# haoheliu/ssr_eval

Hardware: AMD Instinct MI355X
Metric: utterance-pairs/sec (LSD+SSIM, 48kHz, n_fft=2048) (higher is better)
Workload: dtype f64

## Files before the change

ssr_eval_amd/csrc/ssr_stft_wave.h:

```cpp
#pragma once
#include "ssr_stft.h"


constexpr int SSR_W_N = 2048, SSR_W_L = 64, SSR_W_P = 32;
constexpr int SSR_W_TWP = 7 * 32 + 12 * 64;
SSR_DEV int ssr_wpad(int i) { return i + (i >> 5); }
constexpr int SSR_W_PN = SSR_W_N + (SSR_W_N >> 5) + 1;

template <typename T> SSR_DEV cx<T> ssr_w32(int m) {
  constexpr double c[22] = {1.0, 0.98078528040323044913, 0.92387953251128675613, 0.83146961230254523708, 0.70710678118654752440,
                            0.55557023301960222474, 0.38268343236508977173, 0.19509032201612826785, 0.0,
                            -0.19509032201612826785, -0.38268343236508977173, -0.55557023301960222474, -0.70710678118654752440,
                            -0.83146961230254523708, -0.92387953251128675613, -0.98078528040323044913, -1.0,
                            -0.98078528040323044913, -0.92387953251128675613, -0.83146961230254523708, -0.70710678118654752440,
                            -0.55557023301960222474};
  constexpr double s[22] = {0.0, -0.19509032201612826785, -0.38268343236508977173, -0.55557023301960222474, -0.70710678118654752440,
                            -0.83146961230254523708, -0.92387953251128675613, -0.98078528040323044913, -1.0,
                            -0.98078528040323044913, -0.92387953251128675613, -0.83146961230254523708, -0.70710678118654752440,
                            -0.55557023301960222474, -0.38268343236508977173, -0.19509032201612826785, 0.0,
                            0.19509032201612826785, 0.38268343236508977173, 0.55557023301960222474, 0.70710678118654752440,
                            0.83146961230254523708};
  return {(T)c[m], (T)s[m]};
}

template <typename T, int NZ = 32> SSR_DEV void ssr_dft32(cx<T>* v) {
  const T h = (T)0.70710678118654752440;
  static_assert(NZ == 32 || (NZ > 8 && NZ <= 16), "full, or two non-zero row groups");
  SSR_UNROLL for (int n2 = 0; n2 < 8; ++n2) {
    cx<T> t[4] = {v[n2], v[8 + n2], v[16 + n2], v[24 + n2]};
    if (NZ == 32) {
      ssr_bfly4(t);
    } else if (8 + n2 < NZ) {
      const cx<T> r = cmul_negi(t[1]);
      t[2] = csub(t[0], t[1]); t[3] = csub(t[0], r);
      t[1] = cadd(t[0], r);    t[0] = cadd(t[0], v[8 + n2]);
    } else {
      t[1] = t[0]; t[2] = t[0]; t[3] = t[0];
    }
    SSR_UNROLL for (int k1 = 0; k1 < 4; ++k1) {
      const int m = n2 * k1;
      cx<T> x = t[k1];
      if (m == 0) {
      } else if (m == 8) {
        x = cmul_negi(x);
      } else if (m == 16) {
        x = {-x.x, -x.y};
      } else if (m == 4) {
        x = {h * (x.x + x.y), h * (x.y - x.x)};
      } else if (m == 12) {
        x = {h * (x.y - x.x), -h * (x.x + x.y)};
      } else if (m == 20) {
        x = {-h * (x.x + x.y), h * (x.x - x.y)};
      } else {
        x = cmul(x, ssr_w32<T>(m));
      }
      v[8 * k1 + n2] = x;
    }
  }
  SSR_UNROLL for (int k1 = 0; k1 < 4; ++k1) ssr_bfly8(v + 8 * k1);
}
SSR_DEV constexpr int ssr_dft32_freq(int rho) { return (rho >> 3) + 4 * (rho & 7); }

struct SsrTrue { static constexpr bool value = true; };
struct SsrFalse { static constexpr bool value = false; };

template <typename T, bool SUMS> struct SsrWaveRegs {
  cx<T> v[SSR_W_P];
  T tx[SSR_W_P];
  float pa[SSR_W_P], pb[SSR_W_P];
  T wl[SSR_W_P / 2];
  cx<T> tw1[7];
  cx<T> tw2[12];
  double lsd_total;
};

template <typename T, bool SPLIT> struct SsrWaveLds {
  static constexpr size_t bytes() { return sizeof(double) * 4 + sizeof(int) * 8 + sizeof(T) * (SPLIT ? 1 : 2) * SSR_W_PN; }
  double* sc1; int* nz; T* re; T* im;
  SSR_MEMBER explicit SsrWaveLds(char* base) {
    sc1 = reinterpret_cast<double*>(base);
    nz = reinterpret_cast<int*>(sc1 + 4);
    re = reinterpret_cast<T*>(nz + 8);
    im = SPLIT ? re : re + SSR_W_PN;
  }
  SSR_MEMBER bool nonzero(int which, int par) const {
    int f = nz[which * 2 + par];
#ifndef SSR_HOST_EMU
    f = __builtin_amdgcn_readfirstlane(f);
#endif
    return f != 0;
  }
};

template <typename T> struct SsrWaveBuf { T* re; T* im; };

template <typename T, bool SPLIT> constexpr size_t ssr_stft_wave_sums_offset() { return (SsrWaveLds<T, SPLIT>::bytes() + 7) & ~(size_t)7; }
template <typename T, bool SPLIT, bool SUMS> constexpr size_t ssr_stft_wave_lds_bytes() {
  return SUMS ? ssr_stft_wave_sums_offset<T, SPLIT>() + 6 * 64 * sizeof(double) : SsrWaveLds<T, SPLIT>::bytes();
}

struct SsrWaveBase { int st0, ld8, st1; };
SSR_DEV SsrWaveBase ssr_wave_bases(int tid) {
  return {33 * tid, tid + (tid >> 5), 264 * (tid >> 5) + (tid & 31)};
}
SSR_DEV constexpr int ssr_w_off_st0(int i) { return ssr_dft32_freq(i); }
SSR_DEV constexpr int ssr_w_off_ld8(int i) { return 66 * (i >> 3) + 264 * (i & 7); }
SSR_DEV constexpr int ssr_w_off_st1(int i) { return 528 * (i >> 3) + 33 * (i & 7); }

#define SSR_W_EXCHANGE_G(blk, regs, L, WB, WO, RBASES, RIDX, EXTRA)                                       \
  if constexpr (!SPLIT) {                                                                                 \
    SSR_WPHASE(blk, regs, { const int w_ = ssr_wave_bases(tid & 63).WB;                                        \
      SSR_UNROLL for (int i = 0; i < SSR_W_P; ++i) { (L).re[w_ + WO(i)] = R.v[i].x; (L).im[w_ + WO(i)] = R.v[i].y; } }); \
    SSR_WPHASE(blk, regs, { SSR_SCHED_BARRIER(); EXTRA; const auto r_ = RBASES(tid & 63);                    \
      SSR_UNROLL for (int i = 0; i < SSR_W_P; ++i) R.v[i] = {(L).re[RIDX(r_, i)], (L).im[RIDX(r_, i)]}; });   \
  } else {                                                                                                \
    SSR_WPHASE(blk, regs, { const int w_ = ssr_wave_bases(tid & 63).WB;                                        \
      SSR_UNROLL for (int i = 0; i < SSR_W_P; ++i) (L).re[w_ + WO(i)] = R.v[i].x; });                     \
    SSR_WPHASE(blk, regs, { SSR_SCHED_BARRIER(); EXTRA; const auto r_ = RBASES(tid & 63);                    \
      SSR_UNROLL for (int i = 0; i < SSR_W_P; ++i) R.tx[i] = (L).re[RIDX(r_, i)]; });                     \
    SSR_WPHASE(blk, regs, { const int w_ = ssr_wave_bases(tid & 63).WB;                                        \
      SSR_UNROLL for (int i = 0; i < SSR_W_P; ++i) (L).re[w_ + WO(i)] = R.v[i].y; });                     \
    SSR_WPHASE(blk, regs, { const auto r_ = RBASES(tid & 63);                                                \
      SSR_UNROLL for (int i = 0; i < SSR_W_P; ++i) R.v[i] = {R.tx[i], (L).re[RIDX(r_, i)]}; });           \
  }
#define SSR_W_RIDX_LD8(b_, i) ((b_).ld8 + ssr_w_off_ld8(i))
#define SSR_W_EXCHANGE(blk, regs, L, WB, WO, RB, RO, EXTRA) SSR_W_EXCHANGE_G(blk, regs, L, WB, WO, ssr_wave_bases, SSR_W_RIDX_##RB##_##RO, EXTRA)
#define SSR_W_RIDX_ld8_ssr_w_off_ld8(b_, i) SSR_W_RIDX_LD8(b_, i)

struct SsrWavePBase { int ld8, p2, p3; };
SSR_DEV int ssr_wave_pj3(int tid) { return tid == 0 ? 128 : 256 - tid; }
SSR_DEV SsrWavePBase ssr_wave_pbases(int tid) {
  return {tid + (tid >> 5), ssr_wpad(192 - tid), ssr_wpad(ssr_wave_pj3(tid))};
}
SSR_DEV int ssr_w_rd_paired(const SsrWavePBase& B, int i) {
  const int b = i >> 3, q = i & 7;
  return (b == 0 ? B.ld8 : b == 1 ? B.ld8 + 66 : b == 2 ? B.p2 : B.p3) + 264 * q;
}
#define SSR_W_RIDX_PAIRED(b_, i) ssr_w_rd_paired(b_, i)
#define SSR_W_LOAD_TW2_PAIRED { const int t_ = tid & 63; const unsigned l_ = SSR_UIDX(t_);                       \
    const unsigned o2_ = SSR_UIDX(t_ == 0 ? 192 : 64 - t_); const unsigned o3_ = SSR_UIDX(t_ == 0 ? -192 : 64 - t_); \
    SSR_UNROLL for (int i = 0; i < 6; ++i) R.tw2[i] = VT.at(l_ + (SSR_W_N + 224 + 64 * i));                       \
    SSR_UNROLL for (int i = 6; i < 9; ++i) R.tw2[i] = VT.at(o2_ + (SSR_W_N + 224 + 64 * i));                      \
    SSR_UNROLL for (int i = 9; i < 12; ++i) R.tw2[i] = VT.at(o3_ + (SSR_W_N + 224 + 64 * i)); }

#define SSR_W_LOAD_TW1 { const unsigned l_ = SSR_UIDX(tid & 31); \
                         SSR_UNROLL for (int q = 1; q < 8; ++q) R.tw1[q - 1] = VT.at(l_ + (SSR_W_N + 32 * (q - 1))); }
#define SSR_W_LOAD_TW2 { const unsigned l_ = SSR_UIDX(tid & 63); \
                         SSR_UNROLL for (int i = 0; i < 12; ++i) R.tw2[i] = VT.at(l_ + (SSR_W_N + 224 + 64 * i)); }
#define SSR_W_FFT_TAIL(blk, BLK0, regs, L, EXTRA2)                                                                        \
  SSR_W_FFT_TAIL_X(blk, BLK0, regs, L, SSR_W_EXCHANGE(blk, regs, L, st1, ssr_w_off_st1, ld8, ssr_w_off_ld8, SSR_W_LOAD_TW2 EXTRA2))
#define SSR_W_FFT_TAIL_PAIRED(blk, BLK0, regs, L)                                                                         \
  SSR_W_FFT_TAIL_X(blk, BLK0, regs, L, SSR_W_EXCHANGE_G(blk, regs, L, st1, ssr_w_off_st1, ssr_wave_pbases, SSR_W_RIDX_PAIRED, SSR_W_LOAD_TW2_PAIRED))
#define SSR_W_FFT_TAIL_X(blk, BLK0, regs, L, EXCH2)                                                                       \
  blk = BLK0; ssr_launder(blk);                                                                                     \
  SSR_W_EXCHANGE(blk, regs, L, st0, ssr_w_off_st0, ld8, ssr_w_off_ld8, SSR_W_LOAD_TW1);                             \
   \
  SSR_WPHASE(blk, regs, {                                                                                           \
    SSR_UNROLL for (int b = 0; b < 4; ++b) {                                                                        \
      SSR_UNROLL for (int q = 1; q < 8; ++q) R.v[8 * b + q] = cmul(R.v[8 * b + q], R.tw1[q - 1]);                   \
      ssr_bfly8(R.v + 8 * b);                                                                                       \
    }                                                                                                               \
  });                                                                                                               \
  blk = BLK0; ssr_launder(blk);                                                                                     \
  EXCH2;                                                                                                            \
    \
  SSR_WPHASE(blk, regs, {                                                                                           \
    SSR_UNROLL for (int b = 0; b < 4; ++b) {                                                                        \
      cx<T>* x = R.v + 8 * b;                                                                                       \
      const cx<T> w1 = R.tw2[3 * b], w2 = R.tw2[3 * b + 1], w4 = R.tw2[3 * b + 2];                                  \
      x[1] = cmul(x[1], w1);                                                                                        \
      x[2] = cmul(x[2], w2);                                                                                        \
      x[4] = cmul(x[4], w4);                                                                                        \
      const cx<T> w3 = cmul(w1, w2);                                                                                \
      x[3] = cmul(x[3], w3);                                                                                        \
      x[5] = cmul(x[5], cmul(w1, w4));                                                                              \
      x[6] = cmul(x[6], cmul(w2, w4));                                                                              \
      x[7] = cmul(x[7], cmul(w3, w4));                                                                              \
      ssr_bfly8(x);                                                                                                 \
    }                                                                                                               \
  });

template <typename T, int WHICH = 3, typename REGS>
SSR_DEV void ssr_wave_prefetch(const SsrStftParams<T>& p, REGS& R, int tid, const SsrView<float>& va, const SsrView<float>& vb,
                               int u, int n, int n_frames) {
  const int t_c = (u < n_frames) ? u : n_frames - 1;
  const int base = t_c * p.hop - SSR_W_N / 2;
  if (base >= 0 && base + SSR_W_N <= n) {
    SSR_UNROLL for (int r = 0; r < SSR_W_P; ++r) {
      if (WHICH & 1) R.pa[r] = va.at(SSR_UIDX(tid + 64 * r), base);
      if (WHICH & 2) R.pb[r] = vb.at(SSR_UIDX(tid + 64 * r), base);
    }
  } else {
    SSR_UNROLL for (int r = 0; r < SSR_W_P; ++r) {
      const unsigned m = SSR_UIDX(ssr_reflect(base + tid + 64 * r, n));
      if (WHICH & 1) R.pa[r] = va.at(m);
      if (WHICH & 2) R.pb[r] = vb.at(m);
    }
  }
}

template <typename REGS> SSR_DEV void ssr_wave_flags(REGS& R, int tid, int* nz, int par) {
  SSR_UNROLL for (int r = 0; r < SSR_W_P; ++r) { ssr_touch(R.pa[r]); ssr_touch(R.pb[r]); }
  unsigned ora = 0u, orb = 0u;
  SSR_UNROLL for (int r = 1; r < SSR_W_P; ++r) { ora |= ssr_mag_bits(R.pa[r]); orb |= ssr_mag_bits(R.pb[r]); }
  ora |= (tid == 0) ? 0u : ssr_mag_bits(R.pa[0]);
  orb |= (tid == 0) ? 0u : ssr_mag_bits(R.pb[0]);
  SSR_WAVE_ANY_STORE(tid, ora != 0u, nz + par);
  SSR_WAVE_ANY_STORE(tid, orb != 0u, nz + 2 + par);
}

template <typename T, bool SUMS, bool SPLIT, int MAG = -1, typename BLK>
SSR_BODY void ssr_stft_wave_body(const SsrStftParams<T>& p, BLK& blk, int chunk, int item, char* lds_base) {
  constexpr int N = SSR_W_N, F = N / 2 + 1;
  using Regs = SsrWaveRegs<T, SUMS>;
  SsrWaveLds<T, SPLIT> L(lds_base);
  const int n = p.len[item], hop = p.hop;
  const int n_frames = ssr_num_frames_dev(n, N, hop);
  const int S = p.interleave > 1 ? p.interleave : 1;
  const int span0 = (chunk / S) * S * p.units_per_chunk;
  const int u0 = span0 + chunk % S;
  const int u1 = (span0 + S * p.units_per_chunk < n_frames) ? span0 + S * p.units_per_chunk : n_frames;
  const float* sa = p.a + p.a_off[item];
  const float* sb = p.b + p.b_off[item];
  const int64_t row0 = p.frame_off[item];
  double* part = p.part ? p.part + ((int64_t)item * p.n_chunks + chunk) * SSR_NPART : nullptr;
  const int mask = SUMS ? p.metric_mask : (p.metric_mask & SSR_M_LSD);
  const bool want_lsd = mask & SSR_M_LSD;
  const SsrView<float> va(sa, n), vb(sb, n);
  const SsrView<T> vw(p.window, N);
  const SsrView<cx<T>> vt(p.tw, N + SSR_W_TWP);

  double* lsum = reinterpret_cast<double*>(lds_base + ssr_stft_wave_sums_offset<T, SPLIT>());
  SSR_REGS(Regs, regs, blk);
  SSR_WPHASE(blk, regs, {
    R.lsd_total = 0.0;
    if constexpr (SUMS) for (int q = 0; q < 6; ++q) lsum[64 * q + tid] = 0.0;
    if (tid == 0) L.sc1[0] = 0.0;
    if (u0 < u1) {
      ssr_wave_prefetch<T>(p, R, tid, va, vb, u0, n, n_frames);
      SSR_UNROLL for (int r = 0; r < SSR_W_P / 2; ++r) R.wl[r] = vw.at(SSR_UIDX(tid + 64 * r));
    }
    SSR_VMEM_DRAIN();
  });

  BLK blk0 = blk;
  for (int u = u0, it = 0; u < u1; u += S, ++it) {
    blk = blk0; ssr_launder(blk);
    SSR_WPHASE(blk, regs, {
      ssr_wave_flags(R, tid, L.nz, it & 1);
      SSR_UNROLL for (int r = 0; r < SSR_W_P; ++r) {
        const T w = (r < SSR_W_P / 2) ? R.wl[r] : (T)0.5 - R.wl[r - SSR_W_P / 2];
        R.v[r] = {(T)R.pa[r] * w, (T)R.pb[r] * w};
      }
      ssr_dft32(R.v);
      if (want_lsd && it > 0 && tid == 0) R.lsd_total += sqrt(L.sc1[0] / (double)F);
    });
#define VT vt
    SSR_W_FFT_TAIL_PAIRED(blk, blk0, regs, L);
#undef VT

    blk = blk0; ssr_launder(blk);
    const int64_t OP = p.out_pitch ? p.out_pitch : F;
    float* ra0 = p.out_a ? p.out_a + (row0 + u) * OP : nullptr;
    float* rb0 = p.out_b ? p.out_b + (row0 + u) * OP : nullptr;
    SSR_WPHASE(blk, regs, {
      SSR_SCHED_BARRIER();
      double acc[7] = {0.0, 0.0, 0.0, 0.0, 0.0, 0.0, 0.0};
      const int par = it & 1;
      const bool a_nz = L.nonzero(0, par), b_nz = L.nonzero(1, par);
      const bool both = a_nz && b_nz;
      const bool store = MAG < 0 ? p.out_kind == SSR_OUT_MAG : MAG != 0;
      const SsrRwView<float> wa(ra0, store ? F : 0), wb(rb0, (store && rb0 != nullptr) ? F : 0);
      const int lane4 = 4 * tid, lane4_2 = 4 * (192 - tid), lane4_3 = 4 * ssr_wave_pj3(tid);
      auto bin_off = [&](int b, int q) -> int {
        return (b == 0 ? lane4 : b == 1 ? lane4 + 256 : b == 2 ? lane4_2 : lane4_3) + 1024 * q;
      };
      cx<T> rot4 = {(T)0, (T)0};
      if (tid == 0) {
        rot4 = R.v[28];
        const cx<T> t29 = R.v[29], t30 = R.v[30], t31 = R.v[31];
        R.v[31] = R.v[0]; R.v[30] = R.v[7]; R.v[29] = R.v[6]; R.v[28] = R.v[5];
        R.v[7] = t31; R.v[6] = t30; R.v[5] = t29;
      }
      constexpr int G = 2;
      constexpr int PF1 = SUMS ? 1 : 0;
      auto bins = [&](auto fast_tag) {
        constexpr bool FAST = decltype(fast_tag)::value;
        SSR_UNROLL for (int b = 0; b < 4; ++b) SSR_UNROLL for (int q0 = 0; q0 < 4; q0 += G) {
          cx<T> zn[G];
          SSR_UNROLL for (int q = 0; q < G; ++q) zn[q] = R.v[8 * (3 - b) + 7 - (q0 + q)];
          SSR_UNROLL for (int q = 0; q < G; q += 2) {
            const cx<T> zk0 = R.v[8 * b + q0 + q], zk1 = R.v[8 * b + q0 + q + 1];
            f2 e, t;
            if constexpr (FAST) {
              ssr_pair_bins2_fast<T, SUMS>(acc, zk0, zn[q], zk1, zn[q + 1], e, t);
            } else {
              float e0, t0, e1, t1;
              ssr_pair_bin<T, 0, true>(mask, acc, zk0, zn[q], a_nz, b_nz, e0, t0);
              ssr_pair_bin<T, 0, true>(mask, acc, zk1, zn[q + 1], a_nz, b_nz, e1, t1);
              e = f2_make(e0, e1); t = f2_make(t0, t1);
            }
            if (store) {
              wa.st_raw(bin_off(b, q0 + q), e.x);
              wa.st_raw(bin_off(b, q0 + q + 1), e.y);
              wb.st_raw(bin_off(b, q0 + q), t.x);
              wb.st_raw(bin_off(b, q0 + q + 1), t.y);
            }
          }
          if (b == 0 && q0 + G == 4) {
            if (tid == 0) {
              const cx<T> zq = R.v[4];
              float e, t;
              ssr_pair_bin<T, 0, true>(mask, acc, zq, zq, a_nz, b_nz, e, t);
              if (store) { wa.st_raw(4 * (N / 2), e); wb.st_raw(4 * (N / 2), t); }
              R.v[4] = rot4;
            }
          }
          if (b == PF1 && q0 + G == 4) {
            SSR_SCHED_BARRIER();
            ssr_wave_prefetch<T, 1>(p, R, tid, va, vb, u + S, n, n_frames);
            SSR_SCHED_BARRIER();
          }
          if (b == PF1 + 1 && q0 + G == 4) {
            SSR_SCHED_BARRIER();
            ssr_wave_prefetch<T, 2>(p, R, tid, va, vb, u + S, n, n_frames);
            SSR_SCHED_BARRIER();
          }
          if (b == PF1 + 2 && q0 + G == 4) {
            SSR_SCHED_BARRIER();
            SSR_UNROLL for (int r = 0; r < SSR_W_P / 2; ++r) R.wl[r] = vw.at(SSR_UIDX(tid + 64 * r));
            SSR_SCHED_BARRIER();
          }
        }
      };
      constexpr int FULL = SUMS ? (SSR_M_LSD | SSR_M_LOG_SISPEC | SSR_M_SISPEC) : SSR_M_LSD;
      if (both && (mask & 7) == FULL) bins(SsrTrue{});
      else bins(SsrFalse{});
      if (want_lsd) SSR_WAVE_SUM_STORE(tid, 64, acc[0], L.sc1);
      if constexpr (SUMS)
        for (int q = 0; q < 6; ++q) SSR_LDS_ACCUM(lsum + 64 * q + tid, acc[1 + q]);
    });
  }

  if (part == nullptr) return;
  if constexpr (SUMS) {
    for (int q = 0; q < 6; ++q) {
      SSR_WPHASE(blk, regs, SSR_WAVE_SUM_STORE(tid, 64, lsum[64 * q + tid], L.sc1 + 1));
      SSR_WPHASE(blk, regs, if (tid == 0) part[1 + q] = L.sc1[1]);
    }
  } else {
    SSR_WPHASE(blk, regs, if (tid == 0) for (int q = 0; q < 6; ++q) part[1 + q] = 0.0);
  }
  SSR_WPHASE(blk, regs, if (tid == 0) {
    double lsd = R.lsd_total;
    if (want_lsd && u1 > u0) lsd += sqrt(L.sc1[0] / (double)F);
    part[0] = lsd;
    part[7] = 0.0;
  });
}
```

ssr_eval_amd/csrc/tu_stft.inc:

```
#include "ssr_host.h"
#include "ssr_stft_r3.h"
#include "ssr_stft_wave.h"
#include "ssr_stft_rn_wave.h"
#include "ssr_stft_r3_rot.h"

typedef SSR_TU_T TT;
static_assert(SSR_W_N == SSR_WAVE_N && SSR_W_TWP == SSR_WAVE_TWP, "ssr_tables.h appends what ssr_stft_wave.h reads");
static_assert(SSR_W24_N == SSR_WAVE24_N && SSR_W24_TWP == SSR_WAVE24_TWP, "ssr_tables.h appends what ssr_fft24.h reads");

constexpr int ssr_stft_min_waves(int logn, bool blu, bool sums) { return (logn == 11 && !blu && !sums) ? 4 : 1; }

#if SSR_TU_PART <= 2
template <typename T, int LOGN, bool BLU, int MODE, bool SUMS, int E64>
__global__ __launch_bounds__((1 << LOGN) / ssr_stft_ppt(LOGN, BLU), E64 ? 1 : ssr_stft_min_waves(LOGN, BLU, SUMS))
void k_stft(SsrStftParams<T> p) {
  extern __shared__ __attribute__((aligned(16))) char smem[];
  SsrBlk blk{(int)threadIdx.x};
  const int item = blockIdx.x / p.n_chunks, chunk = blockIdx.x % p.n_chunks;
  ssr_stft_body<T, LOGN, BLU, MODE, SUMS, ssr_stft_ppt(LOGN, BLU), E64>(p, blk, chunk, item, smem);
}

template <typename T, int LOGN, bool BLU, int MODE, bool SUMS, int E64 = 0>
static int launch_stft_mode(SsrStftParams<T>& p, int grid, hipStream_t s) {
  constexpr int PPT = ssr_stft_ppt(LOGN, BLU);
  const size_t lds = SsrStftLds<T, LOGN, PPT>::bytes();
  static thread_local SsrLdsSlot slot;
  if (int rc = ssr_allow_lds((const void*)k_stft<T, LOGN, BLU, MODE, SUMS, E64>, lds, &slot)) return rc;
  hipLaunchKernelGGL((k_stft<T, LOGN, BLU, MODE, SUMS, E64>), dim3(grid), dim3((1 << LOGN) / PPT), lds, s, p);
  HIP_TRY(hipGetLastError());
  return SSR_OK;
}

template <typename T, int LOGN, bool BLU> static int launch_stft_inst(SsrStftParams<T>& p, int grid, hipStream_t s) {
  const bool sums = p.metric_mask & (SSR_M_SISPEC | SSR_M_LOG_SISPEC);
  (void)sums;
#if SSR_TU_PART == 2
  return launch_stft_mode<T, LOGN, BLU, SSR_MODE_SINGLE, false>(p, grid, s);
#elif SSR_TU_PART == 1
  if (p.a64 && p.b64)
    return sums ? launch_stft_mode<T, LOGN, BLU, SSR_MODE_PAIR, true, SSR_IN_BOTH64>(p, grid, s)
                : launch_stft_mode<T, LOGN, BLU, SSR_MODE_PAIR, false, SSR_IN_BOTH64>(p, grid, s);
  return sums ? launch_stft_mode<T, LOGN, BLU, SSR_MODE_PAIR, true, SSR_IN_EST64>(p, grid, s)
              : launch_stft_mode<T, LOGN, BLU, SSR_MODE_PAIR, false, SSR_IN_EST64>(p, grid, s);
#else
  return sums ? launch_stft_mode<T, LOGN, BLU, SSR_MODE_PAIR, true>(p, grid, s)
              : launch_stft_mode<T, LOGN, BLU, SSR_MODE_PAIR, false>(p, grid, s);
#endif
}

#if SSR_TU_PART == 0
template <typename T, bool SUMS, bool SPLIT, bool MAG>
__global__ __launch_bounds__(64, SPLIT ? 2 : 1) void k_stft_wave(SsrStftParams<T> p, int n_groups) {
  extern __shared__ __attribute__((aligned(16))) char smem[];
  SsrBlk blk{(int)threadIdx.x};
  int logical = (int)blockIdx.x;
  if (p.interleave > 1) {
    const int S = p.interleave, xcd = (int)blockIdx.x & 7, slot = (int)blockIdx.x >> 3;
    const int G = (slot / S) * 8 + xcd;
    if (G >= n_groups) return;
    logical = G * S + slot % S;
  }
  const int item = logical / p.n_chunks, chunk = logical % p.n_chunks;
  ssr_stft_wave_body<T, SUMS, SPLIT, MAG ? 1 : 0>(p, blk, chunk, item, smem);
}
template <typename T, bool SUMS> static int launch_stft_wave(SsrStftParams<T>& p, int grid, hipStream_t s) {
  const size_t lds = ssr_stft_wave_lds_bytes<T, true, SUMS>();
  int n_groups = grid;
  if (p.interleave > 1) {
    if (p.n_chunks % p.interleave) return ssr_fail(SSR_ERR_INVALID_ARG, "interleaved chunks: n_chunks must be a multiple of the group size");
    n_groups = grid / p.interleave;
    grid = ssr_ceil_div(n_groups, 8) * 8 * p.interleave;
  }
  if (p.out_kind == SSR_OUT_MAG) hipLaunchKernelGGL((k_stft_wave<T, SUMS, true, true>), dim3(grid), dim3(64), lds, s, p, n_groups);
  else hipLaunchKernelGGL((k_stft_wave<T, SUMS, true, false>), dim3(grid), dim3(64), lds, s, p, n_groups);
  HIP_TRY(hipGetLastError());
  return SSR_OK;
}
#endif

static int launch_stft_part(const ssr_plan* pl, SsrStftParams<TT>& p, int grid, hipStream_t s) {
#if SSR_TU_PART == 0
  if (ssr_stft_uses_wave_engine(pl, false)) {
    const bool sums = p.metric_mask & (SSR_M_SISPEC | SSR_M_LOG_SISPEC);
    return sums ? launch_stft_wave<TT, true>(p, grid, s) : launch_stft_wave<TT, false>(p, grid, s);
  }
#endif
#define CASE(L)                                                                   \
  case L:                                                                         \
    return pl->eng.bluestein ? launch_stft_inst<TT, L, true>(p, grid, s) : launch_stft_inst<TT, L, false>(p, grid, s);
  switch (pl->eng.logn) { CASE(8) CASE(9) CASE(10) CASE(11) CASE(12)
    case 13: return launch_stft_inst<TT, 13, true>(p, grid, s);
  }
#undef CASE
  return ssr_fail(SSR_ERR_UNSUPPORTED, "no kernel for this FFT length");
}

#if SSR_TU_PART == 0
template <> int ssr_launch_stft_pair<TT>(const ssr_plan* pl, SsrStftParams<TT>& p, int grid, hipStream_t s) { return launch_stft_part(pl, p, grid, s); }
#elif SSR_TU_PART == 1
template <> int ssr_launch_stft_pair64<TT>(const ssr_plan* pl, SsrStftParams<TT>& p, int grid, hipStream_t s) { return launch_stft_part(pl, p, grid, s); }
#else
template <> int ssr_launch_stft_single<TT>(const ssr_plan* pl, SsrStftParams<TT>& p, int grid, hipStream_t s) { return launch_stft_part(pl, p, grid, s); }
#endif

#else
template <typename T, int LOGN, int MODE, bool SUMS, int E64>
__global__ __launch_bounds__((1 << LOGN) / 8) void k_stft_r3(SsrStftParams<T> p) {
  extern __shared__ __attribute__((aligned(16))) char smem[];
  SsrBlk blk{(int)threadIdx.x};
  const int item = blockIdx.x / p.n_chunks, chunk = blockIdx.x % p.n_chunks;
  ssr_stft_r3_body<T, LOGN, MODE, SUMS, E64>(p, blk, chunk, item, smem);
}

template <typename T, int LOGN, int MODE, bool SUMS, int E64 = 0>
static int launch_stft_r3_mode(SsrStftParams<T>& p, int grid, hipStream_t s) {
  const size_t lds = SsrStftR3Lds<T, LOGN>::bytes(p.n_fft / 3);
  static thread_local SsrLdsSlot slot;
  if (int rc = ssr_allow_lds((const void*)k_stft_r3<T, LOGN, MODE, SUMS, E64>, lds, &slot)) return rc;
  hipLaunchKernelGGL((k_stft_r3<T, LOGN, MODE, SUMS, E64>), dim3(grid), dim3((1 << LOGN) / 8), lds, s, p);
  HIP_TRY(hipGetLastError());
  return SSR_OK;
}

template <typename T, int LOGN> static int launch_stft_r3_inst(SsrStftParams<T>& p, int grid, hipStream_t s) {
  const bool sums = p.metric_mask & (SSR_M_SISPEC | SSR_M_LOG_SISPEC);
  (void)sums;
#if SSR_TU_PART == 3
  if (p.mode != SSR_MODE_PAIR) return launch_stft_r3_mode<T, LOGN, SSR_MODE_SINGLE, false>(p, grid, s);
  return sums ? launch_stft_r3_mode<T, LOGN, SSR_MODE_PAIR, true>(p, grid, s)
              : launch_stft_r3_mode<T, LOGN, SSR_MODE_PAIR, false>(p, grid, s);
#else
  if (p.a64 && p.b64)
    return sums ? launch_stft_r3_mode<T, LOGN, SSR_MODE_PAIR, true, SSR_IN_BOTH64>(p, grid, s)
                : launch_stft_r3_mode<T, LOGN, SSR_MODE_PAIR, false, SSR_IN_BOTH64>(p, grid, s);
  return sums ? launch_stft_r3_mode<T, LOGN, SSR_MODE_PAIR, true, SSR_IN_EST64>(p, grid, s)
              : launch_stft_r3_mode<T, LOGN, SSR_MODE_PAIR, false, SSR_IN_EST64>(p, grid, s);
#endif
}

#if SSR_TU_PART == 3
template <typename T, bool SUMS, int NW, int NQ, int P>
__global__ __launch_bounds__(64 * NW, (NQ == 4 && sizeof(T) == 8) ? 1 : 2) void k_stft_rn_wave(SsrStftParams<T> p) {
  extern __shared__ __attribute__((aligned(16))) char smem[];
  SsrBlk blk{(int)threadIdx.x};
  const int item = blockIdx.x / p.n_chunks, chunk = blockIdx.x % p.n_chunks;
  ssr_stft_rn_wave_body<T, SUMS, NW, NQ, P>(p, blk, chunk, item, smem);
}
template <typename T, bool SUMS, int NW, int NQ, int P> static int launch_stft_rn_wave(SsrStftParams<T>& p, int grid, hipStream_t s) {
  const size_t lds = ssr_stft_rn_wave_lds_bytes<T, NW, SUMS, P>();
  static thread_local SsrLdsSlot slot;
  if (int rc = ssr_allow_lds((const void*)k_stft_rn_wave<T, SUMS, NW, NQ, P>, lds, &slot)) return rc;
  hipLaunchKernelGGL((k_stft_rn_wave<T, SUMS, NW, NQ, P>), dim3(grid), dim3(64 * NW), lds, s, p);
  HIP_TRY(hipGetLastError());
  return SSR_OK;
}
template <typename T, int NW, int NQ, int P> static int launch_stft_rn_wave_sums(SsrStftParams<T>& p, int grid, hipStream_t s) {
  return (p.metric_mask & (SSR_M_SISPEC | SSR_M_LOG_SISPEC)) ? launch_stft_rn_wave<T, true, NW, NQ, P>(p, grid, s)
                                                             : launch_stft_rn_wave<T, false, NW, NQ, P>(p, grid, s);
}
template <typename T, bool SUMS, int NQ, int P, int IN64 = 0>
__global__ __launch_bounds__(64 * SSR_R3ROT_WAVES, 2) void k_stft_r3_rot(SsrStftParams<T> p) {
  extern __shared__ __attribute__((aligned(16))) char smem[];
  SsrBlk blk{(int)threadIdx.x};
  const int item = blockIdx.x / p.n_chunks, chunk = blockIdx.x % p.n_chunks;
  ssr_stft_r3_rot_body<T, SUMS, NQ, P, IN64>(p, blk, chunk, item, smem);
}
template <typename T, bool SUMS, int NQ, int P, int IN64 = 0> static int launch_stft_r3_rot(SsrStftParams<T>& p, int grid, hipStream_t s) {
  const size_t lds = SsrR3RotLds<T, P>::bytes(p.n_fft / 3);
  static thread_local SsrLdsSlot slot;
  if (int rc = ssr_allow_lds((const void*)k_stft_r3_rot<T, SUMS, NQ, P, IN64>, lds, &slot)) return rc;
  hipLaunchKernelGGL((k_stft_r3_rot<T, SUMS, NQ, P, IN64>), dim3(grid), dim3(64 * SSR_R3ROT_WAVES), lds, s, p);
  HIP_TRY(hipGetLastError());
  return SSR_OK;
}
template <> int ssr_launch_stft_rn_wave<TT>(const ssr_plan* pl, SsrStftParams<TT>& p, int grid, hipStream_t s) {
  const bool wide = pl->weng.q > 768;
  if (pl->weng.m == SSR_W24_N) {
    switch (ssr_stft_rn_wave_radix(pl)) {
      case 1: return launch_stft_rn_wave_sums<TT, 1, 3, 24>(p, grid, s);
      case 2: return launch_stft_rn_wave_sums<TT, 2, 3, 24>(p, grid, s);
      case 3: {
        if constexpr (sizeof(TT) == 8) {
          if (p.a64 != nullptr && p.b64 != nullptr)
            return launch_stft_r3_rot<TT, false, 3, 24, SSR_IN_EST64X2>(p, grid, s);
        }
        if (p.a64 != nullptr)
          return (p.metric_mask & (SSR_M_SISPEC | SSR_M_LOG_SISPEC)) ? launch_stft_r3_rot<TT, true, 3, 24, SSR_IN_EST64>(p, grid, s)
                                                                     : launch_stft_r3_rot<TT, false, 3, 24, SSR_IN_EST64>(p, grid, s);
        return (p.metric_mask & (SSR_M_SISPEC | SSR_M_LOG_SISPEC)) ? launch_stft_r3_rot<TT, true, 3, 24>(p, grid, s)
                                                                   : launch_stft_r3_rot<TT, false, 3, 24>(p, grid, s);
      }
    }
    return ssr_fail(SSR_ERR_UNSUPPORTED, "no wave kernel for this n_fft");
  }
  switch (ssr_stft_rn_wave_radix(pl)) {
    case 1: return wide ? launch_stft_rn_wave_sums<TT, 1, 4, 32>(p, grid, s) : launch_stft_rn_wave_sums<TT, 1, 3, 32>(p, grid, s);
    case 2: return wide ? launch_stft_rn_wave_sums<TT, 2, 4, 32>(p, grid, s) : launch_stft_rn_wave_sums<TT, 2, 3, 32>(p, grid, s);
    case 3: return launch_stft_rn_wave_sums<TT, 3, 3, 32>(p, grid, s);
  }
  return ssr_fail(SSR_ERR_UNSUPPORTED, "no wave kernel for this n_fft");
}
#endif

static int launch_stft_r3_part(const ssr_plan* pl, SsrStftParams<TT>& p, int grid, hipStream_t s) {
  switch (pl->eng.logn) {
    case 8: return launch_stft_r3_inst<TT, 8>(p, grid, s);
    case 9: return launch_stft_r3_inst<TT, 9>(p, grid, s);
    case 10: return launch_stft_r3_inst<TT, 10>(p, grid, s);
    case 11: return launch_stft_r3_inst<TT, 11>(p, grid, s);
  }
  return ssr_fail(SSR_ERR_UNSUPPORTED, "no radix-3 kernel for this FFT length");
}
#if SSR_TU_PART == 3
template <> int ssr_launch_stft_r3<TT>(const ssr_plan* pl, SsrStftParams<TT>& p, int grid, hipStream_t s) { return launch_stft_r3_part(pl, p, grid, s); }
#else
template <> int ssr_launch_stft_r3_64<TT>(const ssr_plan* pl, SsrStftParams<TT>& p, int grid, hipStream_t s) { return launch_stft_r3_part(pl, p, grid, s); }
#endif
#endif
```

Baseline: 338,800.

## Pack eight STFT waves per workgroup and share twiddle/window tables in LDS

The wave-engine STFT kernel now launches 512-thread workgroups holding eight independent one-wave chunks, each with its own LDS slice, in place of one 64-thread block per chunk. When capacity allows, the workgroup first copies the twiddle factors and half-window into shared LDS, and the FFT tail and window loads read from there rather than global memory. The goal is to cut repeated global/cache traffic for constant tables and to make CU co-residency of waves explicit. In exchange it adds a workgroup-wide fill phase, requires interleave equal to 8 and chunk counts in multiples of 8, drops the XCD-aware remapping, and may limit occupancy because of the larger per-group LDS footprint.

```diff
diff --git a/ssr_eval_amd/csrc/ssr_stft_wave.h b/ssr_eval_amd/csrc/ssr_stft_wave.h
--- a/ssr_eval_amd/csrc/ssr_stft_wave.h
+++ b/ssr_eval_amd/csrc/ssr_stft_wave.h
@@ -97,6 +97,39 @@
 template <typename T, bool SPLIT> constexpr size_t ssr_stft_wave_sums_offset() { return (SsrWaveLds<T, SPLIT>::bytes() + 7) & ~(size_t)7; }
 template <typename T, bool SPLIT, bool SUMS> constexpr size_t ssr_stft_wave_lds_bytes() {
   return SUMS ? ssr_stft_wave_sums_offset<T, SPLIT>() + 6 * 64 * sizeof(double) : SsrWaveLds<T, SPLIT>::bytes();
+}
+
+constexpr int SSR_WG_WAVES = 8;
+constexpr size_t SSR_LDS_PER_CU = 160 * 1024;
+template <typename T, bool SPLIT, bool SUMS> constexpr size_t ssr_stft_wave_stride() {
+  return (ssr_stft_wave_lds_bytes<T, SPLIT, SUMS>() + 15) & ~(size_t)15;
+}
+template <typename T> constexpr size_t ssr_stft_wave_table_bytes() { return 2 * sizeof(T) * SSR_W_TWP + sizeof(T) * (SSR_W_N / 2); }
+template <typename T, bool SPLIT, bool SUMS> constexpr bool ssr_stft_wave_tables_fit() {
+  return SSR_WG_WAVES * ssr_stft_wave_stride<T, SPLIT, SUMS>() + ssr_stft_wave_table_bytes<T>() <= SSR_LDS_PER_CU;
+}
+template <typename T, bool SPLIT, bool SUMS> constexpr size_t ssr_stft_group_lds_bytes() {
+  return SSR_WG_WAVES * ssr_stft_wave_stride<T, SPLIT, SUMS>() + (ssr_stft_wave_tables_fit<T, SPLIT, SUMS>() ? ssr_stft_wave_table_bytes<T>() : 0);
+}
+template <typename T> struct alignas(2 * sizeof(T)) SsrCxA { T x, y; };
+template <typename T> struct SsrWaveTab {
+  SsrCxA<T>* tw; T* win;
+  SSR_MEMBER explicit SsrWaveTab(char* base) {
+    tw = reinterpret_cast<SsrCxA<T>*>(base);
+    win = reinterpret_cast<T*>(tw + SSR_W_TWP);
+  }
+  SSR_MEMBER cx<T> at(unsigned idx) const { const SsrCxA<T> v = tw[(int)idx - SSR_W_N]; return {v.x, v.y}; }
+};
+template <bool TAB, typename A, typename B> SSR_DEV const auto& ssr_pick_table(const A& lds, const B& global) {
+  if constexpr (TAB) return lds; else return global;
+}
+template <typename T, typename BLK> SSR_BODY void ssr_stft_wave_fill_tables(const SsrStftParams<T>& p, BLK& blk, int nt, char* tab) {
+  const SsrWaveTab<T> W(tab);
+  SSR_REGS(int, regs, blk);
+  SSR_PHASE(blk, regs, {
+    for (int i = tid; i < SSR_W_TWP; i += nt) { const cx<T> v = p.tw[SSR_W_N + i]; W.tw[i] = SsrCxA<T>{v.x, v.y}; }
+    for (int i = tid; i < SSR_W_N / 2; i += nt) W.win[i] = p.window[i];
+  });
 }
 
 struct SsrWaveBase { int st0, ld8, st1; };
@@ -209,8 +242,8 @@
   SSR_WAVE_ANY_STORE(tid, orb != 0u, nz + 2 + par);
 }
 
-template <typename T, bool SUMS, bool SPLIT, int MAG = -1, typename BLK>
-SSR_BODY void ssr_stft_wave_body(const SsrStftParams<T>& p, BLK& blk, int chunk, int item, char* lds_base) {
+template <typename T, bool SUMS, bool SPLIT, int MAG = -1, bool TAB = false, typename BLK>
+SSR_BODY void ssr_stft_wave_body(const SsrStftParams<T>& p, BLK& blk, int chunk, int item, char* lds_base, char* tab = nullptr) {
   constexpr int N = SSR_W_N, F = N / 2 + 1;
   using Regs = SsrWaveRegs<T, SUMS>;
   SsrWaveLds<T, SPLIT> L(lds_base);
@@ -229,6 +262,9 @@
   const SsrView<float> va(sa, n), vb(sb, n);
   const SsrView<T> vw(p.window, N);
   const SsrView<cx<T>> vt(p.tw, N + SSR_W_TWP);
+  const SsrWaveTab<T> wt(tab);
+  const auto& vtx = ssr_pick_table<TAB>(wt, vt);
+#define SSR_W_WIN(m) (TAB ? wt.win[m] : vw.at(SSR_UIDX(m)))
 
   double* lsum = reinterpret_cast<double*>(lds_base + ssr_stft_wave_sums_offset<T, SPLIT>());
   SSR_REGS(Regs, regs, blk);
@@ -238,7 +274,7 @@
     if (tid == 0) L.sc1[0] = 0.0;
     if (u0 < u1) {
       ssr_wave_prefetch<T>(p, R, tid, va, vb, u0, n, n_frames);
-      SSR_UNROLL for (int r = 0; r < SSR_W_P / 2; ++r) R.wl[r] = vw.at(SSR_UIDX(tid + 64 * r));
+      SSR_UNROLL for (int r = 0; r < SSR_W_P / 2; ++r) R.wl[r] = SSR_W_WIN(tid + 64 * r);
     }
     SSR_VMEM_DRAIN();
   });
@@ -255,7 +291,7 @@
       ssr_dft32(R.v);
       if (want_lsd && it > 0 && tid == 0) R.lsd_total += sqrt(L.sc1[0] / (double)F);
     });
-#define VT vt
+#define VT vtx
     SSR_W_FFT_TAIL_PAIRED(blk, blk0, regs, L);
 #undef VT
 
@@ -328,7 +364,7 @@
           }
           if (b == PF1 + 2 && q0 + G == 4) {
             SSR_SCHED_BARRIER();
-            SSR_UNROLL for (int r = 0; r < SSR_W_P / 2; ++r) R.wl[r] = vw.at(SSR_UIDX(tid + 64 * r));
+            SSR_UNROLL for (int r = 0; r < SSR_W_P / 2; ++r) R.wl[r] = SSR_W_WIN(tid + 64 * r);
             SSR_SCHED_BARRIER();
           }
         }
@@ -357,4 +393,5 @@
     part[0] = lsd;
     part[7] = 0.0;
   });
-}
+#undef SSR_W_WIN
+}
diff --git a/ssr_eval_amd/csrc/tu_stft.inc b/ssr_eval_amd/csrc/tu_stft.inc
--- a/ssr_eval_amd/csrc/tu_stft.inc
+++ b/ssr_eval_amd/csrc/tu_stft.inc
@@ -50,31 +50,36 @@
 
 #if SSR_TU_PART == 0
 template <typename T, bool SUMS, bool SPLIT, bool MAG>
-__global__ __launch_bounds__(64, SPLIT ? 2 : 1) void k_stft_wave(SsrStftParams<T> p, int n_groups) {
-  extern __shared__ __attribute__((aligned(16))) char smem[];
-  SsrBlk blk{(int)threadIdx.x};
-  int logical = (int)blockIdx.x;
-  if (p.interleave > 1) {
-    const int S = p.interleave, xcd = (int)blockIdx.x & 7, slot = (int)blockIdx.x >> 3;
-    const int G = (slot / S) * 8 + xcd;
-    if (G >= n_groups) return;
-    logical = G * S + slot % S;
-  }
+__global__ __launch_bounds__(64 * SSR_WG_WAVES) void k_stft_wave(SsrStftParams<T> p, int) {
+  static_assert(SPLIT, "eight one-array blocks per CU");
+  extern __shared__ __attribute__((aligned(16))) char smem[];
+  constexpr bool TAB = ssr_stft_wave_tables_fit<T, SPLIT, SUMS>();
+  constexpr size_t stride = ssr_stft_wave_stride<T, SPLIT, SUMS>();
+  char* tab = smem + SSR_WG_WAVES * stride;
+  if constexpr (TAB) {
+    SsrBlk all{(int)threadIdx.x};
+    ssr_stft_wave_fill_tables<T>(p, all, 64 * SSR_WG_WAVES, tab);
+  }
+  const int wave = __builtin_amdgcn_readfirstlane((int)threadIdx.x) >> 6;
+  SsrBlk blk{(int)threadIdx.x & 63};
+  const int logical = (int)blockIdx.x * SSR_WG_WAVES + wave;
   const int item = logical / p.n_chunks, chunk = logical % p.n_chunks;
-  ssr_stft_wave_body<T, SUMS, SPLIT, MAG ? 1 : 0>(p, blk, chunk, item, smem);
+  ssr_stft_wave_body<T, SUMS, SPLIT, MAG ? 1 : 0, TAB>(p, blk, chunk, item, smem + wave * stride, tab);
+}
+template <typename T, bool SUMS, bool MAG> static int launch_stft_wave_inst(SsrStftParams<T>& p, int n_groups, hipStream_t s) {
+  const size_t lds = ssr_stft_group_lds_bytes<T, true, SUMS>();
+  static thread_local SsrLdsSlot slot;
+  if (int rc = ssr_allow_lds((const void*)k_stft_wave<T, SUMS, true, MAG>, lds, &slot)) return rc;
+  hipLaunchKernelGGL((k_stft_wave<T, SUMS, true, MAG>), dim3(n_groups), dim3(64 * SSR_WG_WAVES), lds, s, p, n_groups);
+  HIP_TRY(hipGetLastError());
+  return SSR_OK;
 }
 template <typename T, bool SUMS> static int launch_stft_wave(SsrStftParams<T>& p, int grid, hipStream_t s) {
-  const size_t lds = ssr_stft_wave_lds_bytes<T, true, SUMS>();
-  int n_groups = grid;
-  if (p.interleave > 1) {
-    if (p.n_chunks % p.interleave) return ssr_fail(SSR_ERR_INVALID_ARG, "interleaved chunks: n_chunks must be a multiple of the group size");
-    n_groups = grid / p.interleave;
-    grid = ssr_ceil_div(n_groups, 8) * 8 * p.interleave;
-  }
-  if (p.out_kind == SSR_OUT_MAG) hipLaunchKernelGGL((k_stft_wave<T, SUMS, true, true>), dim3(grid), dim3(64), lds, s, p, n_groups);
-  else hipLaunchKernelGGL((k_stft_wave<T, SUMS, true, false>), dim3(grid), dim3(64), lds, s, p, n_groups);
-  HIP_TRY(hipGetLastError());
-  return SSR_OK;
+  if (p.interleave != SSR_WG_WAVES || p.n_chunks % SSR_WG_WAVES)
+    return ssr_fail(SSR_ERR_INVALID_ARG, "wave engine: chunks come in whole groups of 8 (one workgroup each)");
+  const int n_groups = grid / SSR_WG_WAVES;
+  return p.out_kind == SSR_OUT_MAG ? launch_stft_wave_inst<T, SUMS, true>(p, n_groups, s)
+                                   : launch_stft_wave_inst<T, SUMS, false>(p, n_groups, s);
 }
 #endif
 
```

Result: slower. 328,000 (-3.2%).
